# rigelshysaj/LaVie

Measured on NVIDIA B200. Metric: denoise steps/s (320x512x16, CFG), higher is better.
Workload: dtype bf16

## Files before the change

### lavie_b200/csrc/gemm.cu

```cuda
#include "common.cuh"

namespace {

constexpr int BLOCK_M = 128;
constexpr int PAIR_M = 256;
constexpr int BLOCK_K = 64;
constexpr int UMMA_K = 16;
constexpr int A_STAGE_BYTES = BLOCK_M * BLOCK_K * 2;
constexpr int NUM_EPI_WARPS = 8;
constexpr int EPI_SPLIT = NUM_EPI_WARPS / 4;
constexpr int NUM_THREADS = 64 + 32 * NUM_EPI_WARPS;
constexpr int EPI_BAR_ID = 1;
constexpr int EPI_CHUNK_BYTES = 32 * 32 * 2;

struct GemmParams {
  int M, N, K;
  int num_k_blocks;
  int k_split_blocks;
  int m_tiles, n_tiles;
  int m_tile0;
  int rows_window;
  int splits, kb_per_split;
  int conv;
  int c_blocks;
  int out_h, out_w, conv_stride;
  int tap_rows;
  int phases;
  int lowres_w;
  int slabs_total;
  const float* bias;
  const float* row_bias;
  int rows_per_batch;
  int ld_row_bias;
  const __nv_bfloat16* residual;
  int ldr;
  int geglu;
  __nv_bfloat16* out;
  int ldo;
  float* partial;
  int* tickets;
  float* colstats;
  int mg8;
  int check;
  int k_rot;
  int debug;
};

template <int BLOCK_N>
struct SmemLayout {
  static constexpr int N_MMA = BLOCK_N > 256 ? 2 : 1;
  static constexpr int UMMA_N = BLOCK_N / N_MMA;
  static constexpr int ACC_STAGES = 2 * BLOCK_N <= 512 ? 2 : 1;
  static constexpr int B_HALF_BYTES = (UMMA_N / 2) * BLOCK_K * 2;
  static constexpr int B_STAGE_BYTES = N_MMA * B_HALF_BYTES;
  static constexpr int STAGE_BYTES = A_STAGE_BYTES + B_STAGE_BYTES;
  static constexpr int BIAS_BYTES = 0;
  static constexpr int EPI_CHUNKS = (BLOCK_N / 32 + EPI_SPLIT - 1) / EPI_SPLIT;
  static constexpr int EPI_BYTES = NUM_EPI_WARPS * EPI_CHUNKS * EPI_CHUNK_BYTES;
  static constexpr int MAX_SMEM = 227 * 1024 - 2048 - BIAS_BYTES - EPI_BYTES;
  static constexpr int STAGES_RAW = MAX_SMEM / STAGE_BYTES;
  static constexpr int STAGES = STAGES_RAW > 8 ? 8 : STAGES_RAW;
  static constexpr int TOTAL = STAGES * STAGE_BYTES + BIAS_BYTES + EPI_BYTES + 1024  + 512 ;
};

__device__ __forceinline__ uint32_t cluster_ctarank() {
  uint32_t r;
  asm volatile("mov.u32 %0, %%cluster_ctarank;" : "=r"(r));
  return r;
}
__device__ __forceinline__ void cluster_sync_all() {
  asm volatile("barrier.cluster.arrive.release.aligned;\n\tbarrier.cluster.wait.acquire.aligned;" ::: "memory");
}
__device__ __forceinline__ uint32_t mapa_u32(uint32_t local_smem_addr, uint32_t rank) {
  uint32_t r;
  asm volatile("mapa.shared::cluster.u32 %0, %1, %2;" : "=r"(r) : "r"(local_smem_addr), "r"(rank));
  return r;
}
__device__ __forceinline__ void mbar_arrive_cluster(uint32_t cluster_addr) {
  asm volatile("mbarrier.arrive.relaxed.cluster.shared::cluster.b64 _, [%0];" ::"r"(cluster_addr) : "memory");
}
__device__ __forceinline__ void tmem_alloc2(uint32_t* slot, uint32_t ncols) {
  asm volatile("tcgen05.alloc.cta_group::2.sync.aligned.shared::cta.b32 [%0], %1;" ::"r"(smem_u32(slot)), "r"(ncols)
               : "memory");
}
__device__ __forceinline__ void tmem_relinquish2() {
  asm volatile("tcgen05.relinquish_alloc_permit.cta_group::2.sync.aligned;" ::: "memory");
}
__device__ __forceinline__ void tmem_dealloc2(uint32_t taddr, uint32_t ncols) {
  asm volatile("tcgen05.dealloc.cta_group::2.sync.aligned.b32 %0, %1;" ::"r"(taddr), "r"(ncols) : "memory");
}
__device__ __forceinline__ void umma2_bf16(uint32_t d_tmem, uint64_t a_desc, uint64_t b_desc, uint32_t idesc,
                                           uint32_t accumulate) {
  asm volatile(
      "{\n\t.reg .pred p;\n\t"
      "setp.ne.b32 p, %4, 0;\n\t"
      "tcgen05.mma.cta_group::2.kind::f16 [%0], %1, %2, %3, p;\n\t}"
      ::"r"(d_tmem), "l"(a_desc), "l"(b_desc), "r"(idesc), "r"(accumulate)
      : "memory");
}
__device__ __forceinline__ void umma2_commit_mc(uint64_t* bar) {
  const uint16_t mask = 3;
  asm volatile(
      "tcgen05.commit.cta_group::2.mbarrier::arrive::one.shared::cluster.multicast::cluster.b64 [%0], %1;"
      ::"r"(smem_u32(bar)), "h"(mask)
      : "memory");
}
__device__ __forceinline__ void tma2_load_2d(void* dst, const CUtensorMap* m, uint32_t bar_cluster_addr, int c0,
                                             int c1) {
  asm volatile(
      "cp.async.bulk.tensor.2d.cta_group::2.shared::cluster.global.mbarrier::complete_tx::bytes [%0], [%1, {%3, %4}], "
      "[%2];" ::"r"(smem_u32(dst)),
      "l"(reinterpret_cast<uint64_t>(m)), "r"(bar_cluster_addr), "r"(c0), "r"(c1)
      : "memory");
}
__device__ __forceinline__ void tma2_load_im2col(void* dst, const CUtensorMap* m, uint32_t bar_cluster_addr, int c,
                                                 int w, int h, int n, uint16_t off_w, uint16_t off_h) {
  asm volatile(
      "cp.async.bulk.tensor.4d.im2col.cta_group::2.shared::cluster.global.mbarrier::complete_tx::bytes [%0], [%1, {%3, "
      "%4, %5, %6}], [%2], {%7, %8};" ::"r"(smem_u32(dst)),
      "l"(reinterpret_cast<uint64_t>(m)), "r"(bar_cluster_addr), "r"(c), "r"(w), "r"(h), "r"(n), "h"(off_w), "h"(off_h)
      : "memory");
}
__device__ __forceinline__ void epi_bar_sync() {
  asm volatile("bar.sync %0, %1;" ::"n"(EPI_BAR_ID), "n"(32 * NUM_EPI_WARPS) : "memory");
}

struct Item {
  int m_blk, n_blk, kb_begin, kb_end, phase;
};
__device__ __forceinline__ Item decode_item(const GemmParams& p, int item) {
  Item it;
  const int split = item % p.splits;
  int rest = item / p.splits;
  it.phase = 0;
  if (p.phases > 1) {
    it.phase = rest % p.phases;
    rest /= p.phases;
  }
  it.n_blk = rest % p.n_tiles;
  it.m_blk = rest / p.n_tiles + p.m_tile0;
  it.kb_begin = split * p.kb_per_split;
  it.kb_end = min(p.num_k_blocks, it.kb_begin + p.kb_per_split);
  return it;
}

template <int BLOCK_N>
__global__ void __cluster_dims__(2, 1, 1) __launch_bounds__(NUM_THREADS, 1)
gemm_bf16_tcgen05(const __grid_constant__ CUtensorMap tmap_a0, const __grid_constant__ CUtensorMap tmap_a1,
                  const __grid_constant__ CUtensorMap tmap_a2, const __grid_constant__ CUtensorMap tmap_a3,
                  const __grid_constant__ CUtensorMap tmap_b, const __grid_constant__ CUtensorMap tmap_out,
                  const __grid_constant__ CUtensorMap tmap_res, const GemmParams p) {
  pdl_launch_dependents();
  using L = SmemLayout<BLOCK_N>;
  constexpr int STAGES = L::STAGES;
  constexpr int ACC_STAGES = L::ACC_STAGES;
  constexpr int ACC_COLS = ACC_STAGES * BLOCK_N;
  constexpr uint32_t TMEM_COLS = (ACC_COLS <= 32) ? 32 : (ACC_COLS <= 64) ? 64 : (ACC_COLS <= 128) ? 128
                                 : (ACC_COLS <= 256) ? 256 : 512;
  static_assert(BLOCK_N % 32 == 0 && BLOCK_N >= 32 && ACC_COLS <= 512 && L::UMMA_N % 16 == 0 && L::UMMA_N <= 256,
                "BLOCK_N");

  extern __shared__ uint8_t smem_raw[];
  uint8_t* smem = reinterpret_cast<uint8_t*>((reinterpret_cast<uintptr_t>(smem_raw) + 1023) & ~uintptr_t(1023));
  uint8_t* s_epi = smem + STAGES * L::STAGE_BYTES + L::BIAS_BYTES;
  uint64_t* full_bar = reinterpret_cast<uint64_t*>(smem + STAGES * L::STAGE_BYTES + L::BIAS_BYTES + L::EPI_BYTES);
  uint64_t* empty_bar = full_bar + STAGES;
  uint64_t* tmem_full = empty_bar + STAGES;
  uint64_t* tmem_empty = tmem_full + 2;
  uint64_t* res_bar = tmem_empty + 2;
  uint32_t* tmem_slot = reinterpret_cast<uint32_t*>(res_bar + NUM_EPI_WARPS);
  volatile uint32_t* s_last = tmem_slot + 1;

  const int warp = threadIdx.x >> 5;
  const int lane = threadIdx.x & 31;
  const uint32_t rank = cluster_ctarank();
  const int pair = blockIdx.x >> 1;
  const int num_pairs = gridDim.x >> 1;
  const int num_items = p.m_tiles * p.n_tiles * p.splits * p.phases;

  if (warp == 0 && lane == 0) {
    tma_prefetch_desc(&tmap_a0);
    tma_prefetch_desc(&tmap_a1);
    if (p.phases > 1) {
      tma_prefetch_desc(&tmap_a2);
      tma_prefetch_desc(&tmap_a3);
    }
    tma_prefetch_desc(&tmap_b);
    tma_prefetch_desc(&tmap_out);
    tma_prefetch_desc(&tmap_res);
    for (int s = 0; s < STAGES; ++s) {
      mbar_init(&full_bar[s], 1);
      mbar_init(&empty_bar[s], 1);
    }
    for (int a = 0; a < 2; ++a) {
      mbar_init(&tmem_full[a], 1);
      mbar_init(&tmem_empty[a], 2 * NUM_EPI_WARPS);
    }
    for (int w = 0; w < NUM_EPI_WARPS; ++w) mbar_init(&res_bar[w], 1);
    mbar_fence_init();
  }
  if (warp == 1) {
    tmem_alloc2(tmem_slot, TMEM_COLS);
    tmem_relinquish2();
  }
  tc_fence_before();
  cluster_sync_all();
  tc_fence_after();
  pdl_wait();
  const uint32_t tmem_base = *tmem_slot;

  if (warp == 0) {
    int stage = 0;
    uint32_t phase = 0;
    for (int item = pair; item < num_items; item += num_pairs) {
      const Item it = decode_item(p, item);
      const int m_cta = it.m_blk * 2 + static_cast<int>(rank);
      const int klen = it.kb_end - it.kb_begin;
      const int rot = (it.m_blk * p.k_rot) % klen;
      for (int i = 0; i < klen; ++i) {
        int kb = it.kb_begin + i + rot;
        if (kb >= it.kb_end) kb -= klen;
        mbar_wait(&empty_bar[stage], phase ^ 1);
        if (elect_one()) {
          uint8_t* a_dst = smem + stage * L::STAGE_BYTES;
          uint8_t* b_dst = a_dst + A_STAGE_BYTES;
          const uint32_t full_leader = mapa_u32(smem_u32(&full_bar[stage]), 0);
          if (p.debug & 1) {
            if (rank == 0) mbar_arrive(&full_bar[stage]);
          } else {
            if (rank == 0) mbar_expect_tx(&full_bar[stage], 2 * L::STAGE_BYTES);
            if (p.conv == 3) {
              const int tap = kb / p.c_blocks;
              const int c0 = (kb - tap * p.c_blocks) * BLOCK_K;
              const int m0 = m_cta * BLOCK_M;
              const int img = m0 / (p.out_h * p.out_w);
              const int rem = m0 - img * (p.out_h * p.out_w);
              const int oy = rem / p.out_w, ox = rem - oy * p.out_w;
              const int px = it.phase & 1, py = it.phase >> 1;
              const CUtensorMap* am = it.phase == 0 ? &tmap_a0 : it.phase == 1 ? &tmap_a1 : it.phase == 2 ? &tmap_a2 : &tmap_a3;
              tma2_load_im2col(a_dst, am, full_leader, c0, ox + px - 1, oy + py - 1, img, static_cast<uint16_t>(tap & 1),
                               static_cast<uint16_t>(tap >> 1));
            } else if (p.conv == 2) {
              const int tap = kb / p.c_blocks;
              tma2_load_2d(a_dst, &tmap_a0, full_leader, (kb - tap * p.c_blocks) * BLOCK_K,
                           m_cta * BLOCK_M + tap * p.tap_rows);
            } else if (p.conv) {
              const int tap = kb / p.c_blocks;
              const int c0 = (kb - tap * p.c_blocks) * BLOCK_K;
              const int m0 = m_cta * BLOCK_M;
              const int img = m0 / (p.out_h * p.out_w);
              const int rem = m0 - img * (p.out_h * p.out_w);
              const int oy = rem / p.out_w, ox = rem - oy * p.out_w;
              tma2_load_im2col(a_dst, &tmap_a0, full_leader, c0, ox * p.conv_stride - 1, oy * p.conv_stride - 1, img,
                               static_cast<uint16_t>(tap % 3), static_cast<uint16_t>(tap / 3));
            } else if (kb < p.k_split_blocks) {
              tma2_load_2d(a_dst, &tmap_a0, full_leader, kb * BLOCK_K, m_cta * BLOCK_M);
            } else {
              tma2_load_2d(a_dst, &tmap_a1, full_leader, (kb - p.k_split_blocks) * BLOCK_K, m_cta * BLOCK_M);
            }
#pragma unroll
            for (int h = 0; h < L::N_MMA; ++h)
              tma2_load_2d(b_dst + h * L::B_HALF_BYTES, &tmap_b, full_leader, kb * BLOCK_K,
                           it.phase * p.N + it.n_blk * BLOCK_N + h * L::UMMA_N + static_cast<int>(rank) * (L::UMMA_N / 2));
          }
        }
        __syncwarp();
        if (++stage == STAGES) { stage = 0; phase ^= 1; }
      }
    }
  } else if (warp == 1) {
    if (rank == 0) {
      constexpr uint32_t idesc = umma_idesc_bf16(PAIR_M, L::UMMA_N, 0, 0);
      int stage = 0;
      uint32_t phase = 0;
      int acc = 0;
      uint32_t acc_phase = 0;
      for (int item = pair; item < num_items; item += num_pairs) {
        const Item it = decode_item(p, item);
        const bool tl = (p.debug & 512) && blockIdx.x == 0 && lane == 0;
        long long* tl_row = reinterpret_cast<long long*>(p.partial) + 8192 + ((item - pair) / num_pairs) * 8;
        if (tl) tl_row[0] = clock64();
        mbar_wait(&tmem_empty[acc], acc_phase ^ 1);
        tc_fence_after();
        if (tl) tl_row[1] = clock64();
        const uint32_t d_tmem = tmem_base + acc * BLOCK_N;
        for (int kb = it.kb_begin; kb < it.kb_end; ++kb) {
          mbar_wait(&full_bar[stage], phase);
          tc_fence_after();
          if (tl && kb == it.kb_begin) tl_row[2] = clock64();
          if (tl && kb == it.kb_end - 1) tl_row[3] = clock64();
          const uint32_t a_addr = smem_u32(smem + stage * L::STAGE_BYTES);
          const uint32_t b_addr = a_addr + A_STAGE_BYTES;
          const uint64_t a_desc = umma_desc_sw128(a_addr, 16, 1024);
          const uint64_t b_desc = umma_desc_sw128(b_addr, 16, 1024);
          if (elect_one()) {
            if (!(p.debug & 2)) {
#pragma unroll
              for (int k = 0; k < BLOCK_K / UMMA_K; ++k) {
#pragma unroll
                for (int h = 0; h < L::N_MMA; ++h)
                  umma2_bf16(d_tmem + h * L::UMMA_N, a_desc + 2 * k, b_desc + h * (L::B_HALF_BYTES >> 4) + 2 * k, idesc,
                             (kb > it.kb_begin || k > 0) ? 1u : 0u);
              }
            }
            umma2_commit_mc(&empty_bar[stage]);
            if (kb == it.kb_end - 1) umma2_commit_mc(&tmem_full[acc]);
          }
          __syncwarp();
          if (++stage == STAGES) { stage = 0; phase ^= 1; }
        }
        if (tl) tl_row[4] = clock64();
        if (++acc == ACC_STAGES) { acc = 0; acc_phase ^= 1; }
      }
    }
  } else {
    const int ew = warp - 2;
    const int q = warp & 3;
    const int chalf = ew >> 2;
    const uint32_t tmem_empty_leader = mapa_u32(smem_u32(&tmem_empty[0]), 0);
    uint8_t* my_stage = s_epi + ew * (L::EPI_CHUNKS * EPI_CHUNK_BYTES);
    uint64_t* my_res_bar = &res_bar[ew];
    uint32_t res_phase = 0;
    const int swz = (lane >> 1) & 3;
    int acc = 0;
    uint32_t acc_phase = 0;
    for (int item = pair; item < num_items; item += num_pairs) {
      const Item it = decode_item(p, item);
      const int split = item % p.splits;
      const int row0 = (it.m_blk * 2 + static_cast<int>(rank)) * BLOCK_M;
      const int wrow0 = row0 + q * 32;
      const int row = wrow0 + lane;
      const bool row_ok = row < p.M;
      const int n0 = it.n_blk * BLOCK_N;
      const bool staged = p.splits == 1 && !p.check;
      const bool fixup = p.splits > 1 && !p.check && p.tickets != nullptr;
      const bool has_res = staged && p.residual != nullptr;
      const bool tl = (p.debug & 512) && blockIdx.x == 0 && ew == 0 && lane == 0;
      long long* tl_row = reinterpret_cast<long long*>(p.partial) + ((item - pair) / num_pairs) * 8;
      if (tl) tl_row[0] = clock64();
      if (staged || fixup) {
        if (lane == 0) asm volatile("cp.async.bulk.wait_group.read 0;" ::: "memory");
        __syncwarp();
      }
      if (staged) {
        if (has_res && lane == 0 && !(p.debug & 64)) {
          int nch = 0;
          for (int c = chalf; c < BLOCK_N / 32; c += EPI_SPLIT) ++nch;
          mbar_expect_tx(my_res_bar, nch * EPI_CHUNK_BYTES);
          int k = 0;
          for (int c = chalf; c < BLOCK_N / 32; c += EPI_SPLIT, ++k)
            tma_load_2d(my_stage + k * EPI_CHUNK_BYTES, &tmap_res, my_res_bar, n0 + c * 32, wrow0);
        }
      }

      if (tl) tl_row[1] = clock64();
      mbar_wait(&tmem_full[acc], acc_phase);
      tc_fence_after();
      if (tl) tl_row[2] = clock64();
      const uint32_t t_row = tmem_base + (static_cast<uint32_t>(q * 32) << 16) + acc * BLOCK_N;
      if (has_res && !(p.debug & 64)) {
        mbar_wait(my_res_bar, res_phase);
        res_phase ^= 1;
      }
      const float* rb_row = (p.row_bias && row_ok) ? p.row_bias + static_cast<size_t>(row / p.rows_per_batch) * p.ld_row_bias
                                                    : nullptr;

      auto stage_and_store = [&](float (&f)[32], int k, int col_out0, bool add_res) {
        uint8_t* buf = my_stage + k * EPI_CHUNK_BYTES + lane * 64;
#pragma unroll
        for (int j = 0; j < 4; ++j) {
          uint4* slot = reinterpret_cast<uint4*>(buf + ((j ^ swz) << 4));
          if (add_res) {
            const uint4 r = *slot;
            const float2 r0 = unpack_bf16(r.x), r1 = unpack_bf16(r.y), r2 = unpack_bf16(r.z), r3 = unpack_bf16(r.w);
            f[8 * j] += r0.x; f[8 * j + 1] += r0.y; f[8 * j + 2] += r1.x; f[8 * j + 3] += r1.y;
            f[8 * j + 4] += r2.x; f[8 * j + 5] += r2.y; f[8 * j + 6] += r3.x; f[8 * j + 7] += r3.y;
          }
          uint4 o;
          o.x = pack_bf16(f[8 * j], f[8 * j + 1]);
          o.y = pack_bf16(f[8 * j + 2], f[8 * j + 3]);
          o.z = pack_bf16(f[8 * j + 4], f[8 * j + 5]);
          o.w = pack_bf16(f[8 * j + 6], f[8 * j + 7]);
          *slot = o;
        }
        fence_proxy_async_smem();
        __syncwarp();
        if (lane == 0 && !(p.debug & 16)) {
          if (p.phases > 1) {
            const int ny0 = wrow0 / p.lowres_w, x0 = wrow0 - ny0 * p.lowres_w;
            asm volatile("cp.async.bulk.tensor.5d.global.shared::cta.bulk_group [%0, {%2, %3, %4, %5, %6}], [%1];" ::"l"(
                             reinterpret_cast<uint64_t>(&tmap_out)),
                         "r"(smem_u32(my_stage + k * EPI_CHUNK_BYTES)), "r"(col_out0), "r"(it.phase & 1), "r"(x0),
                         "r"(it.phase >> 1), "r"(ny0)
                         : "memory");
          } else {
            asm volatile("cp.async.bulk.tensor.2d.global.shared::cta.bulk_group [%0, {%2, %3}], [%1];" ::"l"(
                             reinterpret_cast<uint64_t>(&tmap_out)),
                         "r"(smem_u32(my_stage + k * EPI_CHUNK_BYTES)), "r"(col_out0), "r"(wrow0)
                         : "memory");
          }
          asm volatile("cp.async.bulk.commit_group;" ::: "memory");
        }
      };

      auto chunk_stats = [&](int k, int col_out0) {
        if (col_out0 < p.N && wrow0 < p.M) {
          const int par = lane >> 4, c2 = lane & 15;
          const uint8_t* chunk = my_stage + k * EPI_CHUNK_BYTES;
          float s0 = 0.f, q0 = 0.f;
#pragma unroll
          for (int i = 0; i < 16; ++i) {
            const int r = 2 * i + par;
            const uint32_t w = *reinterpret_cast<const uint32_t*>(chunk + r * 64 + (((c2 >> 2) ^ ((r >> 1) & 3)) << 4) +
                                                                   (c2 & 3) * 4);
            float2 v2 = unpack_bf16(w);
            if (wrow0 + r >= p.M) v2 = make_float2(0.f, 0.f);
            s0 += v2.x + v2.y;
            q0 = fmaf(v2.x, v2.x, fmaf(v2.y, v2.y, q0));
          }
          s0 += __shfl_xor_sync(0xffffffffu, s0, 16);
          q0 += __shfl_xor_sync(0xffffffffu, q0, 16);
          const int col = col_out0 + 2 * c2;
          const int dec = p.mg8 ? (col >> 3) : ((col * 6554) >> 16);
          const int dec0 = p.mg8 ? (col_out0 >> 3) : ((col_out0 * 6554) >> 16);
#pragma unroll
          for (int o = 1; o < 16; o <<= 1) {
            const float ts = __shfl_up_sync(0xffffffffu, s0, o);
            const float tq = __shfl_up_sync(0xffffffffu, q0, o);
            const int td = __shfl_up_sync(0xffffffffu, dec, o);
            if (c2 >= o && td == dec) {
              s0 += ts;
              q0 += tq;
            }
          }
          const int dec_next = __shfl_down_sync(0xffffffffu, dec, 1);
          const bool last_of_piece = (c2 == 15) || (dec_next != dec) || (col + 2 >= p.N);
          if (par == 0 && last_of_piece && col < p.N)
            *reinterpret_cast<float2*>(p.colstats + ((static_cast<size_t>(it.phase * p.slabs_total + (wrow0 >> 5)) * (p.N >> 5) +
                                                      (col_out0 >> 5)) * 4 + (dec - dec0)) * 2) = make_float2(s0, q0);
        }
      };

      if (p.splits > 1 || p.check) {
        float* dst_row = p.partial + (static_cast<size_t>(split) * p.rows_window + (row - p.m_tile0 * PAIR_M)) * p.N;
#pragma unroll 1
        for (int c = chalf; c < BLOCK_N / 32; c += EPI_SPLIT) {
          uint32_t v[32];
          tmem_ld_32x32(t_row + c * 32, v);
          tmem_wait_ld();
          const int col0 = n0 + c * 32;
          if (row_ok) {
#pragma unroll
            for (int j = 0; j < 32; j += 4)
              if (col0 + j < p.N)
                *reinterpret_cast<uint4*>(dst_row + col0 + j) = make_uint4(v[j], v[j + 1], v[j + 2], v[j + 3]);
          }
        }
      } else if (!p.geglu) {
        int k = 0;
#pragma unroll 1
        for (int c = chalf; c < BLOCK_N / 32; c += EPI_SPLIT, ++k) {
          uint32_t v[32];
          tmem_ld_32x32(t_row + c * 32, v);
          tmem_wait_ld();
          if (tl && k == 0) tl_row[3] = clock64();
          const int col0 = n0 + c * 32;
          float f[32];
#pragma unroll
          for (int e = 0; e < 32; ++e) f[e] = __uint_as_float(v[e]);
          if (col0 < p.N) {
            if (p.bias) {
#pragma unroll
              for (int e = 0; e < 32; e += 4) {
                const float4 b4 = __ldg(reinterpret_cast<const float4*>(p.bias + col0 + e));
                f[e] += b4.x; f[e + 1] += b4.y; f[e + 2] += b4.z; f[e + 3] += b4.w;
              }
            }
            if (rb_row) {
#pragma unroll
              for (int e = 0; e < 32; e += 4) {
                const float4 b4 = __ldg(reinterpret_cast<const float4*>(rb_row + col0 + e));
                f[e] += b4.x; f[e + 1] += b4.y; f[e + 2] += b4.z; f[e + 3] += b4.w;
              }
            }
          }
          stage_and_store(f, k, col0, has_res && !(p.debug & 64));
        }
      } else {
        constexpr int HALF = BLOCK_N / 2;
        int k = 0;
#pragma unroll 1
        for (int c = chalf; c < HALF / 32; c += EPI_SPLIT, ++k) {
          uint32_t v[32], g[32];
          tmem_ld_32x32(t_row + c * 32, v);
          tmem_ld_32x32(t_row + HALF + c * 32, g);
          tmem_wait_ld();
          float f[32];
#pragma unroll
          for (int e = 0; e < 32; e += 4) {
            float4 bv = make_float4(0.f, 0.f, 0.f, 0.f), bg = bv;
            if (p.bias) {
              bv = __ldg(reinterpret_cast<const float4*>(p.bias + n0 + c * 32 + e));
              bg = __ldg(reinterpret_cast<const float4*>(p.bias + n0 + HALF + c * 32 + e));
            }
            f[e] = (__uint_as_float(v[e]) + bv.x) * gelu_fast_f(__uint_as_float(g[e]) + bg.x);
            f[e + 1] = (__uint_as_float(v[e + 1]) + bv.y) * gelu_fast_f(__uint_as_float(g[e + 1]) + bg.y);
            f[e + 2] = (__uint_as_float(v[e + 2]) + bv.z) * gelu_fast_f(__uint_as_float(g[e + 2]) + bg.z);
            f[e + 3] = (__uint_as_float(v[e + 3]) + bv.w) * gelu_fast_f(__uint_as_float(g[e + 3]) + bg.w);
          }
          stage_and_store(f, k, it.n_blk * HALF + c * 32, false);
        }
      }
      if (tl) tl_row[4] = clock64();
      tc_fence_before();
      __syncwarp();
      if (lane == 0) mbar_arrive_cluster(tmem_empty_leader + acc * 8);
      bool finished_here = staged;
      if (fixup) {
        epi_bar_sync();
        if (ew == 0 && lane == 0) {
          __threadfence();
          int* tk = p.tickets + (it.m_blk * 2 + static_cast<int>(rank)) * p.n_tiles + it.n_blk;
          const int last = atomicAdd(tk, 1) == p.splits - 1;
          if (last) {
            *tk = 0;
            __threadfence();
          }
          *s_last = static_cast<uint32_t>(last);
        }
        epi_bar_sync();
        if (*s_last) {
          finished_here = true;
          const size_t plane = static_cast<size_t>(p.rows_window) * p.N;
          int k = 0;
#pragma unroll 1
          for (int c = chalf; c < BLOCK_N / 32; c += EPI_SPLIT, ++k) {
            const int col0 = n0 + c * 32;
            const int col = col0 + lane;
            const bool col_ok = col < p.N;
            uint8_t* chunk = my_stage + k * EPI_CHUNK_BYTES;
            const float bias_c = (p.bias && col_ok) ? __ldg(p.bias + col) : 0.f;
            float a[32];
#pragma unroll
            for (int r = 0; r < 32; ++r) a[r] = 0.f;
            const int rows_here = min(32, p.M - wrow0);
            const float* src0 = p.partial + static_cast<size_t>(wrow0 - p.m_tile0 * PAIR_M) * p.N + col;
            if (col_ok) {
              for (int sp = 0; sp < p.splits; ++sp) {
                const float* src = src0 + sp * plane;
#pragma unroll
                for (int r = 0; r < 32; ++r)
                  if (r < rows_here) a[r] += __ldcg(src + static_cast<size_t>(r) * p.N);
              }
            }
#pragma unroll
            for (int r = 0; r < 32; ++r) {
              const int grow = wrow0 + r;
              float v = a[r];
              if (r < rows_here && col_ok) {
                v += bias_c;
                if (p.row_bias) v += __ldg(p.row_bias + static_cast<size_t>(grow / p.rows_per_batch) * p.ld_row_bias + col);
                if (p.residual) v += __bfloat162float(p.residual[static_cast<size_t>(grow) * p.ldr + col]);
              } else {
                v = 0.f;
              }
              *reinterpret_cast<__nv_bfloat16*>(chunk + r * 64 + ((((lane >> 3) ^ ((r >> 1) & 3)) << 4) + (lane & 7) * 2)) =
                  __float2bfloat16_rn(v);
            }
            fence_proxy_async_smem();
            __syncwarp();
            if (lane == 0) {
              asm volatile("cp.async.bulk.tensor.2d.global.shared::cta.bulk_group [%0, {%2, %3}], [%1];" ::"l"(
                               reinterpret_cast<uint64_t>(&tmap_out)),
                           "r"(smem_u32(chunk)), "r"(col0), "r"(wrow0)
                           : "memory");
              asm volatile("cp.async.bulk.commit_group;" ::: "memory");
            }
          }
        }
      }
      if (p.colstats != nullptr && finished_here && !p.check && !p.geglu) {
        int k = 0;
        for (int c = chalf; c < BLOCK_N / 32; c += EPI_SPLIT, ++k) chunk_stats(k, n0 + c * 32);
      }
      if (tl) tl_row[5] = clock64();
      if (++acc == ACC_STAGES) { acc = 0; acc_phase ^= 1; }
    }
  }

  if (warp >= 2 && lane == 0) asm volatile("cp.async.bulk.wait_group 0;" ::: "memory");
  tc_fence_before();
  cluster_sync_all();
  if (warp == 1) {
    tc_fence_after();
    tmem_dealloc2(tmem_base, TMEM_COLS);
  }
}

__global__ void __launch_bounds__(256)
splitk_reduce_kernel(const float* __restrict__ partial, int splits, int M, int N, const float* __restrict__ bias,
                     const float* __restrict__ row_bias, int rows_per_batch, int ld_row_bias,
                     const __nv_bfloat16* __restrict__ residual, int ldr, __nv_bfloat16* __restrict__ out, int ldo,
                     int row0) {
  pdl_prologue();
  const int nvec = N >> 2;
  const long long total = static_cast<long long>(M) * nvec;
  for (long long i = blockIdx.x * static_cast<long long>(blockDim.x) + threadIdx.x; i < total;
       i += static_cast<long long>(gridDim.x) * blockDim.x) {
    const int row = static_cast<int>(i / nvec);
    const int col = static_cast<int>(i % nvec) * 4;
    float4 a = *reinterpret_cast<const float4*>(partial + static_cast<size_t>(row) * N + col);
    for (int s = 1; s < splits; ++s) {
      const float4 b = *reinterpret_cast<const float4*>(partial + (static_cast<size_t>(s) * M + row) * N + col);
      a.x += b.x; a.y += b.y; a.z += b.z; a.w += b.w;
    }
    if (bias) {
      const float4 b = *reinterpret_cast<const float4*>(bias + col);
      a.x += b.x; a.y += b.y; a.z += b.z; a.w += b.w;
    }
    if (row_bias) {
      const float4 b = *reinterpret_cast<const float4*>(row_bias + static_cast<size_t>((row + row0) / rows_per_batch) * ld_row_bias + col);
      a.x += b.x; a.y += b.y; a.z += b.z; a.w += b.w;
    }
    if (residual) {
      const uint2 r = *reinterpret_cast<const uint2*>(residual + static_cast<size_t>(row) * ldr + col);
      const float2 r0 = unpack_bf16(r.x), r1 = unpack_bf16(r.y);
      a.x += r0.x; a.y += r0.y; a.z += r1.x; a.w += r1.y;
    }
    *reinterpret_cast<uint2*>(out + static_cast<size_t>(row) * ldo + col) = make_uint2(pack_bf16(a.x, a.y), pack_bf16(a.z, a.w));
  }
}

__global__ void __launch_bounds__(256)
splitk_reduce_stats_kernel(const float* __restrict__ partial, int splits, int M, int N, int M_total,
                           const float* __restrict__ bias, const float* __restrict__ row_bias, int rows_per_batch,
                           int ld_row_bias, const __nv_bfloat16* __restrict__ residual, int ldr,
                           __nv_bfloat16* __restrict__ out, int ldo, int row0, float* __restrict__ colstats, int mg) {
  pdl_prologue();
  constexpr int R = 4;
  __shared__ float s_cs[8][128][2];
  const int tx = threadIdx.x & 31, ty = threadIdx.x >> 5;
  const int cbase = blockIdx.y * 128;
  const int col = cbase + tx * 4;
  const int r_begin = blockIdx.x * 32 + ty * R;
  float s[4] = {0.f, 0.f, 0.f, 0.f}, q[4] = {0.f, 0.f, 0.f, 0.f};
  if (col < N) {
    float4 b4 = make_float4(0.f, 0.f, 0.f, 0.f);
    if (bias) b4 = *reinterpret_cast<const float4*>(bias + col);
    float4 acc[R];
#pragma unroll
    for (int i = 0; i < R; ++i) {
      const int row = r_begin + i;
      acc[i] = row < M ? *reinterpret_cast<const float4*>(partial + static_cast<size_t>(row) * N + col) : b4;
    }
    for (int sp = 1; sp < splits; ++sp) {
#pragma unroll
      for (int i = 0; i < R; ++i) {
        const int row = r_begin + i;
        if (row < M) {
          const float4 b = *reinterpret_cast<const float4*>(partial + (static_cast<size_t>(sp) * M + row) * N + col);
          acc[i].x += b.x; acc[i].y += b.y; acc[i].z += b.z; acc[i].w += b.w;
        }
      }
    }
#pragma unroll
    for (int i = 0; i < R; ++i) {
      const int row = r_begin + i;
      if (row >= M) continue;
      float4 a = acc[i];
      a.x += b4.x; a.y += b4.y; a.z += b4.z; a.w += b4.w;
      if (row_bias) {
        const float4 b = *reinterpret_cast<const float4*>(row_bias + static_cast<size_t>((row + row0) / rows_per_batch) * ld_row_bias + col);
        a.x += b.x; a.y += b.y; a.z += b.z; a.w += b.w;
      }
      if (residual) {
        const uint2 r = *reinterpret_cast<const uint2*>(residual + static_cast<size_t>(row) * ldr + col);
        const float2 r0 = unpack_bf16(r.x), r1 = unpack_bf16(r.y);
        a.x += r0.x; a.y += r0.y; a.z += r1.x; a.w += r1.y;
      }
      const uint2 o = make_uint2(pack_bf16(a.x, a.y), pack_bf16(a.z, a.w));
      *reinterpret_cast<uint2*>(out + static_cast<size_t>(row) * ldo + col) = o;
      if (row + row0 < M_total) {
        const float2 v0 = unpack_bf16(o.x), v1 = unpack_bf16(o.y);
        s[0] += v0.x; q[0] = fmaf(v0.x, v0.x, q[0]);
        s[1] += v0.y; q[1] = fmaf(v0.y, v0.y, q[1]);
        s[2] += v1.x; q[2] = fmaf(v1.x, v1.x, q[2]);
        s[3] += v1.y; q[3] = fmaf(v1.y, v1.y, q[3]);
      }
    }
  }
#pragma unroll
  for (int e = 0; e < 4; ++e) {
    s_cs[ty][tx * 4 + e][0] = s[e];
    s_cs[ty][tx * 4 + e][1] = q[e];
  }
  __syncthreads();
  if (threadIdx.x < 16) {
    const int cl = threadIdx.x >> 2, piece = threadIdx.x & 3;
    const int c0 = cbase + cl * 32;
    if (c0 < N) {
      const int dec = c0 / mg + piece;
      const int lo = max(c0, dec * mg), hi = min(min(c0 + 32, dec * mg + mg), N);
      if (lo < hi) {
        float a = 0.f, b = 0.f;
        for (int c = lo; c < hi; ++c)
#pragma unroll
          for (int g = 0; g < 8; ++g) {
            a += s_cs[g][c - cbase][0];
            b += s_cs[g][c - cbase][1];
          }
        const size_t slab = static_cast<size_t>((blockIdx.x * 32 + row0) >> 5);
        *reinterpret_cast<float2*>(colstats + ((slab * (N >> 5) + (c0 >> 5)) * 4 + piece) * 2) = make_float2(a, b);
      }
    }
  }
}

__global__ void __launch_bounds__(256)
splitk_reduce_check_kernel(const float* __restrict__ partial, int splits, int M, int N, const float* __restrict__ bias,
                           const float* __restrict__ row_bias, int rows_per_batch, int ld_row_bias,
                           const __nv_bfloat16* __restrict__ residual, int ldr, int geglu,
                           __nv_bfloat16* __restrict__ out, int ldo, int row0) {
  pdl_prologue();
  const int n_out = geglu ? N / 2 : N;
  const long long total = static_cast<long long>(M) * n_out;
  for (long long i = blockIdx.x * static_cast<long long>(blockDim.x) + threadIdx.x; i < total;
       i += static_cast<long long>(gridDim.x) * blockDim.x) {
    const int row = static_cast<int>(i / n_out);
    const int col = static_cast<int>(i - static_cast<long long>(row) * n_out);
    auto acc_at = [&](int c) {
      float a = partial[static_cast<size_t>(row) * N + c];
      for (int s = 1; s < splits; ++s) a += partial[(static_cast<size_t>(s) * M + row) * N + c];
      if (bias) a += bias[c];
      return a;
    };
    float v;
    if (geglu) {
      const int t = col >> 7, j = col & 127;
      const float val = acc_at(t * 256 + j), gate = acc_at(t * 256 + 128 + j);
      v = val * (0.5f * gate * (1.0f + erff(gate * 0.70710678118654752440f)));
    } else {
      v = acc_at(col);
      if (row_bias) v += row_bias[static_cast<size_t>((row + row0) / rows_per_batch) * ld_row_bias + col];
      if (residual) {
        const __nv_bfloat16* r = residual + static_cast<size_t>(row) * ldr + col;
        v += __bfloat162float(r[0]) + __bfloat162float(r[N]);
      }
    }
    const __nv_bfloat16 hi = __float2bfloat16_rn(v);
    const __nv_bfloat16 lo = __float2bfloat16_rn(v - __bfloat162float(hi));
    __nv_bfloat16* o = out + static_cast<size_t>(row) * ldo + col;
    o[0] = hi;
    o[n_out] = lo;
    o[2 * n_out] = hi;
  }
}

template <int BLOCK_N>
int launch_gemm(const CUtensorMap& a0, const CUtensorMap& a1, const CUtensorMap& a2, const CUtensorMap& a3,
                const CUtensorMap& b, const CUtensorMap& mo, const CUtensorMap& mr, const GemmParams& p,
                int num_sms, cudaStream_t stream) {
  using L = SmemLayout<BLOCK_N>;
  static LavieSmemConfig configured;
  int rc = lavie_config_smem(gemm_bf16_tcgen05<BLOCK_N>, L::TOTAL, &configured, "gemm_bf16_tcgen05");
  if (rc) return rc;
  const int items = p.m_tiles * p.n_tiles * p.splits * p.phases;
  int pairs = num_sms / 2;
  if (items < pairs) pairs = items;
  launch_pdl(gemm_bf16_tcgen05<BLOCK_N>, 2 * pairs, NUM_THREADS, L::TOTAL, stream, a0, a1, a2, a3, b, mo, mr, p);
  rc = lavie_check_launch("gemm_bf16_tcgen05");
  if (rc) return rc;
  if (p.check) {
    const int row0 = p.m_tile0 * PAIR_M;
    const long long total = static_cast<long long>(p.rows_window) * (p.geglu ? p.N / 2 : p.N);
    long long blocks = (total + 255) / 256;
    if (blocks > 148 * 16) blocks = 148 * 16;
    launch_pdl(splitk_reduce_check_kernel, static_cast<int>(blocks), 256, 0, stream, p.partial, p.splits, p.rows_window,
               p.N, p.bias, p.row_bias, p.rows_per_batch, p.ld_row_bias,
               p.residual ? p.residual + static_cast<size_t>(row0) * p.ldr : nullptr, p.ldr, p.geglu,
               p.out + static_cast<size_t>(row0) * p.ldo, p.ldo, row0);
    rc = lavie_check_launch("splitk_reduce_check_kernel");
  } else if (p.splits > 1 && p.tickets != nullptr) {
  } else if (p.splits > 1 && p.colstats != nullptr) {
    const int row0 = p.m_tile0 * PAIR_M;
    dim3 grid((p.rows_window + 31) / 32, (p.N + 127) / 128);
    launch_pdl(splitk_reduce_stats_kernel, grid, 256, 0, stream, p.partial, p.splits, p.rows_window, p.N, p.M, p.bias,
               p.row_bias, p.rows_per_batch, p.ld_row_bias,
               p.residual ? p.residual + static_cast<size_t>(row0) * p.ldr : nullptr, p.ldr,
               p.out + static_cast<size_t>(row0) * p.ldo, p.ldo, row0, p.colstats, p.mg8 ? 8 : 10);
    rc = lavie_check_launch("splitk_reduce_stats_kernel");
  } else if (p.splits > 1) {
    const int row0 = p.m_tile0 * PAIR_M;
    const long long total = static_cast<long long>(p.rows_window) * (p.N >> 2);
    long long blocks = (total + 255) / 256;
    if (blocks > 148 * 8) blocks = 148 * 8;
    launch_pdl(splitk_reduce_kernel, static_cast<int>(blocks), 256, 0, stream, p.partial, p.splits, p.rows_window, p.N,
               p.bias, p.row_bias, p.rows_per_batch, p.ld_row_bias,
               p.residual ? p.residual + static_cast<size_t>(row0) * p.ldr : nullptr, p.ldr,
               p.out + static_cast<size_t>(row0) * p.ldo, p.ldo, row0);
    rc = lavie_check_launch("splitk_reduce_kernel");
  }
  return rc;
}

int g_force_splits = 0;
int g_debug = 0;
int g_k_rot = 0;
int g_no_tail = 0;
int g_inkernel_reduce = 0;
constexpr size_t TICKET_BYTES = 64 * 1024;
int num_sms() { return lavie_num_sms(); }

struct Plan {
  int bn;
  int splits, kb_per_split;
  int tail_tiles;
  int tail_splits, tail_kb_per_split;
};

double window_cost(int m_tiles, int n_tiles, int bn, int s, int kbps, double t_kb, double t_epi, int pairs, int N) {
  const long items = static_cast<long>(m_tiles) * n_tiles * s;
  const long waves = (items + pairs - 1) / pairs;
  double cost = static_cast<double>(waves) * (kbps * t_kb + 1500.0 + 6.0 * bn + t_epi);
  if (s > 1) cost += 4000.0 + 0.0013 * (s + 0.5) * static_cast<double>(m_tiles) * PAIR_M * N;
  return cost;
}

double best_split(int m_tiles, int n_tiles, int bn, int num_k_blocks, int max_splits, double t_kb, double t_epi,
                  int pairs, int N, size_t ws_bytes, int forced, int* s_out, int* kbps_out) {
  double best = 1e30;
  const long tiles = static_cast<long>(m_tiles) * n_tiles;
  for (int s = 1; s <= max_splits; ++s) {
    if (s > 1) {
      if (static_cast<size_t>(s) * m_tiles * PAIR_M * N * 4 > ws_bytes) break;
      if (num_k_blocks / s < 8) break;
      if (tiles * (s - 1) >= pairs) break;
    }
    if (forced && s != forced) continue;
    const int kbps = (num_k_blocks + s - 1) / s;
    if ((num_k_blocks + kbps - 1) / kbps != s) continue;
    const double c = window_cost(m_tiles, n_tiles, bn, s, kbps, t_kb, t_epi, pairs, N);
    if (c < best) {
      best = c;
      *s_out = s;
      *kbps_out = kbps;
    }
  }
  return best;
}

Plan make_plan(int M, int N, int num_k_blocks, int forced_bn, bool geglu, bool conv, size_t ws_bytes,
               bool no_split = false) {
  const int pairs = num_sms() / 2;
  const int m_tiles = (M + PAIR_M - 1) / PAIR_M;
  const int cands[6] = {320, 256, 192, 160, 128, 64};
  Plan best{128, 1, num_k_blocks, 0, 1, num_k_blocks};
  double best_cost = 1e30;
  const int max_splits = (geglu || no_split) ? 1 : 16;
  const int forced_s = (geglu || no_split) ? 0 : g_force_splits;
  for (int i = 0; i < 6; ++i) {
    const int bn = cands[i];
    if (forced_bn && bn != forced_bn) continue;
    if (geglu && bn != 256) continue;
    const int n_tiles = (N + bn - 1) / bn;
    const double t_kb = fmax(2.0 * bn, (16384.0 + 64.0 * bn) / (conv ? 38.0 : 47.0));
    const double t_epi = bn > 256 ? 5000.0 : 0.0;
    int s = 1, kbps = num_k_blocks;
    const double c1 = best_split(m_tiles, n_tiles, bn, num_k_blocks, max_splits, t_kb, t_epi, pairs, N, ws_bytes,
                                 forced_s, &s, &kbps);
    if (c1 < best_cost) {
      best_cost = c1;
      best = Plan{bn, s, kbps, 0, 1, num_k_blocks};
    }
    const long tiles = static_cast<long>(m_tiles) * n_tiles;
    if (geglu || no_split || forced_s || g_no_tail || tiles <= pairs || num_k_blocks < 16) continue;
    for (int tail = 1; tail < m_tiles && tail <= 16; ++tail) {
      const int main_tiles = m_tiles - tail;
      const long main_items = static_cast<long>(main_tiles) * n_tiles;
      if (main_items % pairs != 0 && main_items % pairs < pairs * 3 / 4) continue;
      int ts = 1, tk = num_k_blocks;
      const double ct = best_split(tail, n_tiles, bn, num_k_blocks, 16, t_kb, t_epi, pairs, N, ws_bytes, 0, &ts, &tk);
      const double cm = window_cost(main_tiles, n_tiles, bn, 1, num_k_blocks, t_kb, t_epi, pairs, N);
      const double c2 = cm + ct + 6000.0;
      if (c2 < 0.93 * best_cost) {
        best_cost = c2;
        best = Plan{bn, 1, num_k_blocks, tail, ts, tk};
      }
    }
// ... 379 lines not shown
```

Before: 46.97.

## Pipeline epilogue residual loads per chunk with per-chunk barriers and partial store waits

Replaces the single per-warp residual barrier with one mbarrier per epilogue chunk. The old code waited for all prior TMA stores to drain before issuing any residual loads. The new code waits only until the store occupying each chunk's buffer has been read, then loads that chunk, and each chunk waits on its own residual barrier before being consumed. This overlaps outstanding output stores with residual loads and epilogue math, at the cost of more barrier state and more complex phase tracking.

Measured after the change: 46.57 (median of 6 runs). About the same (-0.9%).

```diff
diff --git a/lavie_b200/csrc/gemm.cu b/lavie_b200/csrc/gemm.cu
--- a/lavie_b200/csrc/gemm.cu
+++ b/lavie_b200/csrc/gemm.cu
@@ -54,13 +54,15 @@
   static constexpr int B_HALF_BYTES = (UMMA_N / 2) * BLOCK_K * 2;
   static constexpr int B_STAGE_BYTES = N_MMA * B_HALF_BYTES;
   static constexpr int STAGE_BYTES = A_STAGE_BYTES + B_STAGE_BYTES;
-  static constexpr int BIAS_BYTES = 0;
   static constexpr int EPI_CHUNKS = (BLOCK_N / 32 + EPI_SPLIT - 1) / EPI_SPLIT;
   static constexpr int EPI_BYTES = NUM_EPI_WARPS * EPI_CHUNKS * EPI_CHUNK_BYTES;
-  static constexpr int MAX_SMEM = 227 * 1024 - 2048 - BIAS_BYTES - EPI_BYTES;
+  static constexpr int MAX_SMEM = 227 * 1024 - 2048 - EPI_BYTES;
   static constexpr int STAGES_RAW = MAX_SMEM / STAGE_BYTES;
   static constexpr int STAGES = STAGES_RAW > 8 ? 8 : STAGES_RAW;
-  static constexpr int TOTAL = STAGES * STAGE_BYTES + BIAS_BYTES + EPI_BYTES + 1024  + 512 ;
+  static constexpr int BAR_BYTES = 512;
+  static constexpr int TOTAL = STAGES * STAGE_BYTES + EPI_BYTES + 1024  + BAR_BYTES;
+  static_assert((2 * STAGES + 4 + NUM_EPI_WARPS * EPI_CHUNKS) * 8 + 8 <= BAR_BYTES, "barrier area");
+  static_assert(TOTAL <= 227 * 1024, "shared memory per block");
 };
 
 __device__ __forceinline__ uint32_t cluster_ctarank() {
@@ -123,6 +125,15 @@
 }
 __device__ __forceinline__ void epi_bar_sync() {
   asm volatile("bar.sync %0, %1;" ::"n"(EPI_BAR_ID), "n"(32 * NUM_EPI_WARPS) : "memory");
+}
+__device__ __forceinline__ void bulk_wait_read_pending(int n) {
+  switch (n) {
+    case 0: asm volatile("cp.async.bulk.wait_group.read 0;" ::: "memory"); break;
+    case 1: asm volatile("cp.async.bulk.wait_group.read 1;" ::: "memory"); break;
+    case 2: asm volatile("cp.async.bulk.wait_group.read 2;" ::: "memory"); break;
+    case 3: asm volatile("cp.async.bulk.wait_group.read 3;" ::: "memory"); break;
+    default: asm volatile("cp.async.bulk.wait_group.read 4;" ::: "memory"); break;
+  }
 }
 
 struct Item {
@@ -159,16 +170,17 @@
                                  : (ACC_COLS <= 256) ? 256 : 512;
   static_assert(BLOCK_N % 32 == 0 && BLOCK_N >= 32 && ACC_COLS <= 512 && L::UMMA_N % 16 == 0 && L::UMMA_N <= 256,
                 "BLOCK_N");
+  static_assert(L::EPI_CHUNKS <= 5, "bulk_wait_read_pending covers at most 4 groups in flight");
 
   extern __shared__ uint8_t smem_raw[];
   uint8_t* smem = reinterpret_cast<uint8_t*>((reinterpret_cast<uintptr_t>(smem_raw) + 1023) & ~uintptr_t(1023));
-  uint8_t* s_epi = smem + STAGES * L::STAGE_BYTES + L::BIAS_BYTES;
-  uint64_t* full_bar = reinterpret_cast<uint64_t*>(smem + STAGES * L::STAGE_BYTES + L::BIAS_BYTES + L::EPI_BYTES);
+  uint8_t* s_epi = smem + STAGES * L::STAGE_BYTES;
+  uint64_t* full_bar = reinterpret_cast<uint64_t*>(s_epi + L::EPI_BYTES);
   uint64_t* empty_bar = full_bar + STAGES;
   uint64_t* tmem_full = empty_bar + STAGES;
   uint64_t* tmem_empty = tmem_full + 2;
   uint64_t* res_bar = tmem_empty + 2;
-  uint32_t* tmem_slot = reinterpret_cast<uint32_t*>(res_bar + NUM_EPI_WARPS);
+  uint32_t* tmem_slot = reinterpret_cast<uint32_t*>(res_bar + NUM_EPI_WARPS * L::EPI_CHUNKS);
   volatile uint32_t* s_last = tmem_slot + 1;
 
   const int warp = threadIdx.x >> 5;
@@ -196,7 +208,7 @@
       mbar_init(&tmem_full[a], 1);
       mbar_init(&tmem_empty[a], 2 * NUM_EPI_WARPS);
     }
-    for (int w = 0; w < NUM_EPI_WARPS; ++w) mbar_init(&res_bar[w], 1);
+    for (int s = 0; s < NUM_EPI_WARPS * L::EPI_CHUNKS; ++s) mbar_init(&res_bar[s], 1);
     mbar_fence_init();
   }
   if (warp == 1) {
@@ -319,8 +331,11 @@
     const int chalf = ew >> 2;
     const uint32_t tmem_empty_leader = mapa_u32(smem_u32(&tmem_empty[0]), 0);
     uint8_t* my_stage = s_epi + ew * (L::EPI_CHUNKS * EPI_CHUNK_BYTES);
-    uint64_t* my_res_bar = &res_bar[ew];
+    uint64_t* my_res_bar = &res_bar[ew * L::EPI_CHUNKS];
     uint32_t res_phase = 0;
+    const bool staged = p.splits == 1 && !p.check;
+    const bool use_res = staged && p.residual != nullptr && !(p.debug & 64);
+    const int n_store = ((p.geglu ? BLOCK_N / 2 : BLOCK_N) / 32 - chalf + EPI_SPLIT - 1) / EPI_SPLIT;
     const int swz = (lane >> 1) & 3;
     int acc = 0;
     uint32_t acc_phase = 0;
@@ -332,24 +347,15 @@
       const int row = wrow0 + lane;
       const bool row_ok = row < p.M;
       const int n0 = it.n_blk * BLOCK_N;
-      const bool staged = p.splits == 1 && !p.check;
       const bool fixup = p.splits > 1 && !p.check && p.tickets != nullptr;
-      const bool has_res = staged && p.residual != nullptr;
       const bool tl = (p.debug & 512) && blockIdx.x == 0 && ew == 0 && lane == 0;
       long long* tl_row = reinterpret_cast<long long*>(p.partial) + ((item - pair) / num_pairs) * 8;
       if (tl) tl_row[0] = clock64();
-      if (staged || fixup) {
-        if (lane == 0) asm volatile("cp.async.bulk.wait_group.read 0;" ::: "memory");
-        __syncwarp();
-      }
-      if (staged) {
-        if (has_res && lane == 0 && !(p.debug & 64)) {
-          int nch = 0;
-          for (int c = chalf; c < BLOCK_N / 32; c += EPI_SPLIT) ++nch;
-          mbar_expect_tx(my_res_bar, nch * EPI_CHUNK_BYTES);
-          int k = 0;
-          for (int c = chalf; c < BLOCK_N / 32; c += EPI_SPLIT, ++k)
-            tma_load_2d(my_stage + k * EPI_CHUNK_BYTES, &tmap_res, my_res_bar, n0 + c * 32, wrow0);
+      if (use_res && lane == 0) {
+        for (int k = 0; k < n_store; ++k) {
+          bulk_wait_read_pending(n_store - 1 - k);
+          mbar_expect_tx(&my_res_bar[k], EPI_CHUNK_BYTES);
+          tma_load_2d(my_stage + k * EPI_CHUNK_BYTES, &tmap_res, &my_res_bar[k], n0 + (chalf + k * EPI_SPLIT) * 32, wrow0);
         }
       }
 
@@ -358,14 +364,16 @@
       tc_fence_after();
       if (tl) tl_row[2] = clock64();
       const uint32_t t_row = tmem_base + (static_cast<uint32_t>(q * 32) << 16) + acc * BLOCK_N;
-      if (has_res && !(p.debug & 64)) {
-        mbar_wait(my_res_bar, res_phase);
-        res_phase ^= 1;
-      }
       const float* rb_row = (p.row_bias && row_ok) ? p.row_bias + static_cast<size_t>(row / p.rows_per_batch) * p.ld_row_bias
                                                     : nullptr;
 
       auto stage_and_store = [&](float (&f)[32], int k, int col_out0, bool add_res) {
+        if (add_res) {
+          mbar_wait(&my_res_bar[k], res_phase);
+        } else {
+          if (lane == 0) bulk_wait_read_pending(n_store - 1);
+          __syncwarp();
+        }
         uint8_t* buf = my_stage + k * EPI_CHUNK_BYTES + lane * 64;
 #pragma unroll
         for (int j = 0; j < 4; ++j) {
@@ -484,7 +492,7 @@
               }
             }
           }
-          stage_and_store(f, k, col0, has_res && !(p.debug & 64));
+          stage_and_store(f, k, col0, use_res);
         }
       } else {
         constexpr int HALF = BLOCK_N / 2;
@@ -539,6 +547,8 @@
             const int col = col0 + lane;
             const bool col_ok = col < p.N;
             uint8_t* chunk = my_stage + k * EPI_CHUNK_BYTES;
+            if (lane == 0) bulk_wait_read_pending(n_store - 1);
+            __syncwarp();
             const float bias_c = (p.bias && col_ok) ? __ldg(p.bias + col) : 0.f;
             float a[32];
 #pragma unroll
@@ -584,6 +594,7 @@
         for (int c = chalf; c < BLOCK_N / 32; c += EPI_SPLIT, ++k) chunk_stats(k, n0 + c * 32);
       }
       if (tl) tl_row[5] = clock64();
+      if (use_res) res_phase ^= 1;
       if (++acc == ACC_STAGES) { acc = 0; acc_phase ^= 1; }
     }
   }
```
